# aiqm/torchani

Measured on AMD Instinct MI355X. Metric: atom*steps/sec (energy+forces) ANI-2x, higher is better.
Workload: dtype f32; 1 GPU; ANI-2x 8-member ensemble, 2336064-atom periodic water box (0.1 atoms/A^3), energy+forces, seeded random weights; n_atoms=2336064, shuffled_input=False, evaluated_on_cell_sorted_copy=False, two_product_backward=False

## Files before the change

torchani_amd/csrc/nbr.hip:

```cpp
#include "anihip_common.h"

namespace anihip {

struct GridDesc {
    double cell[9];
    double inv[9];
    double f0[3];
    double sc[3];
    float step[9];
    int nb[3];
    int range[3];
    int rep[3];
    int pbc[3];
    int ncell;
    unsigned lo_enc[3], hi_enc[3];
};

struct NbrWorkspace {
    GridDesc *desc;
    float4 *pos4;
    int *cellid;
    int *sorted_idx;
    float4 *pos4s;
    int *cell_start;
    int *cell_fill;
    int *scan_tmp;
};

static inline size_t align256(size_t x) { return (x + 255) & ~(size_t)255; }

static size_t carve(NbrWorkspace *w, char *base, int64_t n, int64_t max_cells)
{
    size_t off = 0;
    auto take = [&](size_t bytes) {
        char *p = base ? base + off : nullptr;
        off += align256(bytes);
        return p;
    };
    GridDesc *desc = (GridDesc *)take(sizeof(GridDesc));
    float4 *pos4 = (float4 *)take(sizeof(float4) * (size_t)n);
    int *cellid = (int *)take(sizeof(int) * (size_t)n);
    int *sorted_idx = (int *)take(sizeof(int) * (size_t)n);
    float4 *pos4s = (float4 *)take(sizeof(float4) * (size_t)n);
    int *cell_start = (int *)take(sizeof(int) * (size_t)(max_cells + 1));
    int *cell_fill = (int *)take(sizeof(int) * (size_t)(max_cells + 1));
    int *scan_tmp = (int *)take(sizeof(int) * (size_t)(max_cells / 1024 + 4));
    if (w) *w = NbrWorkspace{desc, pos4, cellid, sorted_idx, pos4s, cell_start, cell_fill, scan_tmp};
    return off;
}

__device__ __forceinline__ unsigned enc_f(float f)
{
    unsigned u = __float_as_uint(f);
    return (u & 0x80000000u) ? ~u : (u | 0x80000000u);
}
__device__ __forceinline__ float dec_f(unsigned e)
{
    unsigned u = (e & 0x80000000u) ? (e & 0x7FFFFFFFu) : ~e;
    return __uint_as_float(u);
}

__device__ void inv3(const double *m, double *o)
{
    double a = m[0], b = m[1], c = m[2], d = m[3], e = m[4], f = m[5], g = m[6], h = m[7], i = m[8];
    double det = a * (e * i - f * h) - b * (d * i - f * g) + c * (d * h - e * g);
    double id = 1.0 / det;
    o[0] = (e * i - f * h) * id; o[1] = (c * h - b * i) * id; o[2] = (b * f - c * e) * id;
    o[3] = (f * g - d * i) * id; o[4] = (a * i - c * g) * id; o[5] = (c * d - a * f) * id;
    o[6] = (d * h - e * g) * id; o[7] = (b * g - a * h) * id; o[8] = (a * e - b * d) * id;
}


__device__ void desc_fill(GridDesc *g, const float *cell, int pbc_mask, float cutoff)
{
    for (int q = 0; q < 9; ++q) g->cell[q] = cell ? (double)cell[q] : ((q % 4 == 0) ? 1.0 : 0.0);
    inv3(g->cell, g->inv);
    for (int k = 0; k < 3; ++k) {
        g->pbc[k] = (cell && ((pbc_mask >> k) & 1)) ? 1 : 0;
        double nrm = sqrt(g->inv[0 + k] * g->inv[0 + k] + g->inv[3 + k] * g->inv[3 + k] +
                          g->inv[6 + k] * g->inv[6 + k]);
        g->rep[k] = g->pbc[k] ? (int)ceil((double)cutoff * nrm) : 0;
        g->lo_enc[k] = 0xFFFFFFFFu;
        g->hi_enc[k] = 0u;
        g->f0[k] = 0.0;
        g->sc[k] = 1.0;
        g->nb[k] = 1;
        g->range[k] = 0;
    }
    g->ncell = 1;
}

__global__ void k_desc_init(GridDesc *g, const float *cell, int pbc_mask, float cutoff, uint32_t *status)
{
    if (blockIdx.x != 0) return;
    if (threadIdx.x < ANIHIP_STATUS_WORDS) status[threadIdx.x] = 0u;
    if (threadIdx.x == 0) desc_fill(g, cell, pbc_mask, cutoff);
}

__global__ void k_bbox(GridDesc *g, int64_t n, const int32_t *species, const float *coords)
{
    float lo[3] = {3.0e38f, 3.0e38f, 3.0e38f}, hi[3] = {-3.0e38f, -3.0e38f, -3.0e38f};
    for (int64_t i = blockIdx.x * (int64_t)blockDim.x + threadIdx.x; i < n;
         i += (int64_t)gridDim.x * blockDim.x) {
        if (species[i] < 0) continue;
        double x = coords[3 * i], y = coords[3 * i + 1], z = coords[3 * i + 2];
        for (int k = 0; k < 3; ++k) {
            float f = (float)(x * g->inv[0 + k] + y * g->inv[3 + k] + z * g->inv[6 + k]);
            lo[k] = fminf(lo[k], f);
            hi[k] = fmaxf(hi[k], f);
        }
    }
    for (int k = 0; k < 3; ++k) {
        for (int o = 32; o > 0; o >>= 1) {
            lo[k] = fminf(lo[k], __shfl_xor(lo[k], o));
            hi[k] = fmaxf(hi[k], __shfl_xor(hi[k], o));
        }
        if (lane_id() == 0) {
            atomicMin(&g->lo_enc[k], enc_f(lo[k]));
            atomicMax(&g->hi_enc[k], enc_f(hi[k]));
        }
    }
}

__global__ void k_grid_setup(GridDesc *g, float cutoff, int64_t max_cells, uint32_t *status)
{
    if (threadIdx.x != 0 || blockIdx.x != 0) return;
    double h[3], span[3];
    for (int k = 0; k < 3; ++k) {
        double nrm = sqrt(g->inv[0 + k] * g->inv[0 + k] + g->inv[3 + k] * g->inv[3 + k] +
                          g->inv[6 + k] * g->inv[6 + k]);
        h[k] = 1.0 / nrm;
        if (g->pbc[k]) {
            span[k] = 1.0;
            g->f0[k] = 0.0;
        } else {
            double lo = (double)dec_f(g->lo_enc[k]), hi = (double)dec_f(g->hi_enc[k]);
            if (!(hi >= lo)) { lo = 0.0; hi = 0.0; }
            double pad = 1e-4 * nrm + 1e-6 * (fabs(lo) + fabs(hi));
            lo -= pad; hi += pad;
            span[k] = hi - lo;
            g->f0[k] = lo;
        }
        int nb = (int)floor(span[k] * h[k] / (double)cutoff);
        g->nb[k] = nb < 1 ? 1 : nb;
    }
    bool coarsened = false;
    while ((int64_t)g->nb[0] * g->nb[1] * g->nb[2] > max_cells) {
        int k = 0;
        if (g->nb[1] > g->nb[k]) k = 1;
        if (g->nb[2] > g->nb[k]) k = 2;
        g->nb[k] = (g->nb[k] + 1) / 2;
        coarsened = true;
    }
    if (coarsened) atomicOr(&status[0], ANIHIP_ST_GRID_OVERFLOW);
    for (int k = 0; k < 3; ++k) {
        g->sc[k] = (double)g->nb[k] / span[k];
        double width = span[k] * h[k] / g->nb[k];
        g->range[k] = g->pbc[k] ? (int)ceil((double)cutoff / width) : 1;
        for (int q = 0; q < 3; ++q) g->step[3 * k + q] = (float)(g->cell[3 * k + q] / g->sc[k]);
    }
    g->ncell = g->nb[0] * g->nb[1] * g->nb[2];
    status[2] = (uint32_t)g->ncell;
}


__global__ void k_prep_batch(GridDesc *g, int64_t n, const int32_t *species, const float *coords, float4 *pos4,
                             const float *cell, int pbc_mask, float cutoff, uint32_t *status)
{
    if (blockIdx.x == 0) {
        if (threadIdx.x < ANIHIP_STATUS_WORDS) status[threadIdx.x] = 0u;
        if (threadIdx.x == 0) desc_fill(g, cell, pbc_mask, cutoff);
    }
    int64_t i = blockIdx.x * (int64_t)blockDim.x + threadIdx.x;
    if (i >= n) return;
    float x = coords[3 * i], y = coords[3 * i + 1], z = coords[3 * i + 2];
    if (cell && (pbc_mask & 7)) {
        double c[9], inv[9], f[3];
        for (int q = 0; q < 9; ++q) c[q] = (double)cell[q];
        inv3(c, inv);
        for (int k = 0; k < 3; ++k) {
            f[k] = (double)x * inv[0 + k] + (double)y * inv[3 + k] + (double)z * inv[6 + k];
            if ((pbc_mask >> k) & 1) f[k] -= floor(f[k]);
        }
        x = (float)(f[0] * c[0] + f[1] * c[3] + f[2] * c[6]);
        y = (float)(f[0] * c[1] + f[1] * c[4] + f[2] * c[7]);
        z = (float)(f[0] * c[2] + f[1] * c[5] + f[2] * c[8]);
    }
    int sp = species[i];
    uint32_t w = ((uint32_t)i & IDX_MASK) | ((sp < 0 ? SP_PAD : (uint32_t)sp) << 28);
    pos4[i] = make_float4(x, y, z, __uint_as_float(w));
}


__device__ __forceinline__ int wave_runs(int key, int &rank, int &head)
{
    const int lane = lane_id();
    const int k = key < 0 ? -1 - lane : key;
    const int prev = __shfl_up(k, 1);
    const bool is_head = lane == 0 || k != prev;
    const uint64_t heads = __ballot(is_head);
    const uint64_t below = heads & ((lane == 63) ? ~0ull : ((2ull << lane) - 1ull));
    head = 63 - (int)__builtin_clzll(below);
    rank = lane - head;
    const uint64_t above = lane == 63 ? 0ull : (heads >> (lane + 1));
    const int next = above ? lane + 1 + (int)__builtin_ctzll(above) : 64;
    return (is_head && key >= 0) ? next - lane : 0;
}

__global__ void k_bin_count(const GridDesc *g, int64_t n, const int32_t *species, const float *coords,
                            float4 *pos4, int *cellid, int *cell_cnt)
{
    int64_t i = blockIdx.x * (int64_t)blockDim.x + threadIdx.x;
    int c = -1;
    if (i < n) {
        int sp = species[i];
        if (sp >= 0) {
            double x = coords[3 * i], y = coords[3 * i + 1], z = coords[3 * i + 2];
            int b[3];
            double loc[3];
            for (int k = 0; k < 3; ++k) {
                double f = x * g->inv[0 + k] + y * g->inv[3 + k] + z * g->inv[6 + k];
                if (g->pbc[k]) f -= floor(f);
                double q = (f - g->f0[k]) * g->sc[k];
                int bk = (int)floor(q);
                bk = bk < 0 ? 0 : (bk >= g->nb[k] ? g->nb[k] - 1 : bk);
                b[k] = bk;
                loc[k] = (q - bk) / g->sc[k];
            }
            float ox = (float)(loc[0] * g->cell[0] + loc[1] * g->cell[3] + loc[2] * g->cell[6]);
            float oy = (float)(loc[0] * g->cell[1] + loc[1] * g->cell[4] + loc[2] * g->cell[7]);
            float oz = (float)(loc[0] * g->cell[2] + loc[1] * g->cell[5] + loc[2] * g->cell[8]);
            uint32_t w = ((uint32_t)i & IDX_MASK) | ((uint32_t)sp << 28);
            pos4[i] = make_float4(ox, oy, oz, __uint_as_float(w));
            c = (b[0] * g->nb[1] + b[1]) * g->nb[2] + b[2];
        }
        cellid[i] = c;
    }
    int rank, head;
    const int run = wave_runs(c, rank, head);
    if (run > 0) atomicAdd(&cell_cnt[c], run);
}

__global__ void k_scan_local(const GridDesc *g, const int *in, int *out, int *block_sums)
{
    __shared__ int s[1024];
    const int n = g->ncell;
    int i = blockIdx.x * 1024 + threadIdx.x;
    if (blockIdx.x * 1024 >= n + 1) return;
    int v = (i < n) ? in[i] : 0;
    s[threadIdx.x] = v;
    __syncthreads();
    for (int o = 1; o < 1024; o <<= 1) {
        int t = (threadIdx.x >= o) ? s[threadIdx.x - o] : 0;
        __syncthreads();
        s[threadIdx.x] += t;
        __syncthreads();
    }
    if (i <= n) out[i] = s[threadIdx.x] - v;
    if (threadIdx.x == 1023) block_sums[blockIdx.x] = s[1023];
}

__global__ __launch_bounds__(1024) void k_scan_top(const GridDesc *g, int *block_sums)
{
    __shared__ int s[1024];
    __shared__ int carry;
    if (blockIdx.x != 0) return;
    const int nblk = (g->ncell + 1 + 1023) / 1024;
    if (threadIdx.x == 0) carry = 0;
    __syncthreads();
    for (int base = 0; base < nblk; base += 1024) {
        const int i = base + (int)threadIdx.x;
        const int v = i < nblk ? block_sums[i] : 0;
        s[threadIdx.x] = v;
        __syncthreads();
        for (int o = 1; o < 1024; o <<= 1) {
            const int t = (threadIdx.x >= (unsigned)o) ? s[threadIdx.x - o] : 0;
            __syncthreads();
            s[threadIdx.x] += t;
            __syncthreads();
        }
        if (i < nblk) block_sums[i] = carry + s[threadIdx.x] - v;
        __syncthreads();
        if (threadIdx.x == 1023) carry += s[1023];
        __syncthreads();
    }
}

__global__ void k_scan_add(const GridDesc *g, int *out, const int *block_sums)
{
    int i = blockIdx.x * 1024 + threadIdx.x;
    if (i <= g->ncell) out[i] += block_sums[blockIdx.x];
}

__global__ void k_bin_fill(int64_t n, const int *cellid, const int *cell_start, int *cell_fill,
                           int *sorted_idx)
{
    int64_t i = blockIdx.x * (int64_t)blockDim.x + threadIdx.x;
    const int c = i < n ? cellid[i] : -1;
    int rank, head;
    const int run = wave_runs(c, rank, head);
    int base = 0;
    if (run > 0) base = atomicAdd(&cell_fill[c], run);
    base = __shfl(base, head);
    if (c >= 0) sorted_idx[cell_start[c] + base + rank] = (int)i;
}

__global__ void k_bin_rank_gather(int64_t n, const int *cellid, const int *cell_start, const int *sorted_idx,
                                  const float4 *pos4, float4 *pos4s)
{
    const int64_t i = blockIdx.x * (int64_t)blockDim.x + threadIdx.x;
    if (i >= n) return;
    const int c = cellid[i];
    if (c < 0) return;
    const int b = cell_start[c], e = cell_start[c + 1];
    int rank = 0;
    for (int p = b; p < e; ++p) rank += sorted_idx[p] < (int)i ? 1 : 0;
    pos4s[b + rank] = pos4[i];
}


constexpr int NBR_WPB = 4;

__device__ __forceinline__ int wrap_bin(int c, int nb)
{
    c = c < 0 ? c + nb : c;
    c = c >= nb ? c - nb : c;
    if (c < 0 || c >= nb) c = ((c % nb) + nb) % nb;
    return c;
}

struct HitList {
    float4 *buf;
    int n;
    bool overflow;
};

__device__ __forceinline__ void push_hits(HitList &h, bool hit, float dx, float dy, float dz, float w)
{
    uint64_t m = __ballot(hit);
    if (m == 0) return;
    int pos = h.n + mbcnt(m);
    if (hit && pos < MAXR) h.buf[pos] = make_float4(dx, dy, dz, w);
    h.n += __popcll(m);
    if (h.n > MAXR) {
        h.overflow = true;
        h.n = MAXR;
    }
}

__device__ void emit_row(HitList &h, int S, float rca2, int row_cap, uint32_t *meta_i, float4 *row,
                         uint32_t *status)
{
    wave_sync();
    const int lane = lane_id();
    int cnt[2][MAX_S];
#pragma unroll
    for (int g = 0; g < 2; ++g)
#pragma unroll
        for (int t = 0; t < MAX_S; ++t) cnt[g][t] = 0;
    const int n = h.n;
    for (int b0 = 0; b0 < n; b0 += WAVE) {
        int e = b0 + lane;
        bool v = e < n;
        float4 q = h.buf[v ? e : 0];
        int grp = (q.x * q.x + q.y * q.y + q.z * q.z <= rca2) ? 0 : 1;
        int sp = (int)(__float_as_uint(q.w) >> 28);
#pragma unroll
        for (int g = 0; g < 2; ++g)
#pragma unroll
            for (int t = 0; t < MAX_S; ++t)
                if (t < S) cnt[g][t] += __popcll(__ballot(v && grp == g && sp == t));
    }
    int nA = 0, nF = 0, mx = 0;
#pragma unroll
    for (int t = 0; t < MAX_S; ++t) {
        nA += cnt[0][t];
        nF += cnt[1][t];
        mx = max(mx, max(cnt[0][t], cnt[1][t]));
    }
    bool bad = h.overflow || (nA + nF > row_cap) || nA > MAXA || mx > 255;
    if (bad) {
// ... 56 lines not shown
        const size_t row0 = (size_t)(i - lo) * row_cap;
        if (lane == 0) meta_i[0] = (uint32_t)row0;
        const float4 pi = pos4[i];
        if ((__float_as_uint(pi.w) >> 28) == SP_PAD) {
            if (lane == 0) { meta_i[1] = 0; meta_i[2] = 0; meta_i[3] = 0; meta_i[4] = 0; meta_i[5] = 0; }
            continue;
        }
        HitList h{s_hits[wib], 0, false};
        const int64_t mol0 = (i / A) * A;
        for (int n0 = -r0; n0 <= r0; ++n0)
            for (int n1 = -r1; n1 <= r1; ++n1)
                for (int n2 = -r2; n2 <= r2; ++n2) {
                    const float sx = (float)(n0 * g->cell[0] + n1 * g->cell[3] + n2 * g->cell[6]);
                    const float sy = (float)(n0 * g->cell[1] + n1 * g->cell[4] + n2 * g->cell[7]);
                    const float sz = (float)(n0 * g->cell[2] + n1 * g->cell[5] + n2 * g->cell[8]);
                    const bool central_img = (n0 == 0 && n1 == 0 && n2 == 0);
                    for (int a0 = 0; a0 < A; a0 += WAVE) {
                        int a = a0 + lane;
                        bool v = a < A;
                        float4 c = pos4[mol0 + (v ? a : 0)];
                        float dx = (c.x + sx) - pi.x, dy = (c.y + sy) - pi.y, dz = (c.z + sz) - pi.z;
                        float d2 = dx * dx + dy * dy + dz * dz;
                        bool hit = v && ((__float_as_uint(c.w) >> 28) != SP_PAD) && d2 <= rcr2 &&
                                   !(central_img && (mol0 + a) == i);
                        push_hits(h, hit, dx, dy, dz, c.w);
                    }
                }
        emit_row(h, S, rca2, row_cap, meta_i, ent + row0, status);
        wave_sync();
    }
}

__global__ __launch_bounds__(NBR_WPB * WAVE) void k_nbr_cell(
    const GridDesc *g, int S, float rcr2, float rca2, int64_t lo, int64_t hi, const float4 *pos4,
    const int *cellid, const int *cell_start, const float4 *pos4s, int row_cap, uint32_t *meta,
    float4 *ent, uint32_t *status, const int *handled, const int *n_unhandled)
{
    if (n_unhandled && blockIdx.x == 0 && threadIdx.x == 0) status[3] = (uint32_t)*n_unhandled;
    if (n_unhandled && *n_unhandled == 0) return;
    __shared__ float4 s_hits[NBR_WPB][MAXR];
    __shared__ int s_pend[NBR_WPB][WAVE];
    __shared__ int s_k0[NBR_WPB][WAVE];
    __shared__ float4 s_shift[NBR_WPB][WAVE];
    const int wib = threadIdx.x >> 6, lane = lane_id();
    int *pend = s_pend[wib], *k0t = s_k0[wib];
    float4 *shift = s_shift[wib];
    const int64_t nw = (int64_t)gridDim.x * NBR_WPB;
    const int nb0 = g->nb[0], nb1 = g->nb[1], nb2 = g->nb[2];
    const int R0 = g->range[0], R1 = g->range[1], R2 = g->range[2];
    const int p0 = g->pbc[0], p1 = g->pbc[1], p2 = g->pbc[2];
    float st[9];
#pragma unroll
    for (int q = 0; q < 9; ++q) st[q] = g->step[q];
    const int n1 = 2 * R1 + 1, n2 = 2 * R2 + 1, ncells = (2 * R0 + 1) * n1 * n2;
    const float inv_n2 = 1.0f / (float)n2, inv_n1 = 1.0f / (float)n1;
    for (int64_t i = lo + blockIdx.x * (int64_t)NBR_WPB + wib; i < hi; i += nw) {
        uint32_t *meta_i = meta + (size_t)i * META_W;
        const size_t row0 = (size_t)(i - lo) * row_cap;
        if (lane == 0) meta_i[0] = (uint32_t)row0;
        const int c = cellid[i];
        if (c < 0) {
            if (lane == 0) { meta_i[1] = 0; meta_i[2] = 0; meta_i[3] = 0; meta_i[4] = 0; meta_i[5] = 0; }
            continue;
        }
        if (handled && handled[c]) continue;
        const float4 pi = pos4[i];
        const int cu = uniform(c);
        const int b2 = cu % nb2, b1 = (cu / nb2) % nb1, b0 = cu / (nb2 * nb1);
        HitList h{s_hits[wib], 0, false};
        for (int cb = 0; cb < ncells; cb += WAVE) {
            const int ci = cb + lane;
            const int q2 = (int)(((float)ci + 0.5f) * inv_n2);
            const int q1 = (int)(((float)q2 + 0.5f) * inv_n1);
            const int o2 = ci - q2 * n2 - R2, o1 = q2 - q1 * n1 - R1, o0 = q1 - R0;
            int c0 = b0 + o0, c1 = b1 + o1, c2 = b2 + o2;
            bool ok = ci < ncells;
            if (p0) c0 = wrap_bin(c0, nb0); else ok = ok && c0 >= 0 && c0 < nb0;
            if (p1) c1 = wrap_bin(c1, nb1); else ok = ok && c1 >= 0 && c1 < nb1;
            if (p2) c2 = wrap_bin(c2, nb2); else ok = ok && c2 >= 0 && c2 < nb2;
            const int cw = ok ? (c0 * nb1 + c1) * nb2 + c2 : 0;
            const int kbeg = cell_start[cw], kend = cell_start[cw + 1];
            const int cnt = ok ? kend - kbeg : 0;
            int incl = cnt;
#pragma unroll
            for (int d = 1; d < WAVE; d <<= 1) {
                const int up = __shfl_up(incl, d);
                incl += lane >= d ? up : 0;
            }
            const int total = __builtin_amdgcn_readlane(incl, WAVE - 1);
            pend[lane] = incl;
            k0t[lane] = kbeg - (incl - cnt);
            shift[lane] = make_float4(o0 * st[0] + o1 * st[3], o0 * st[1] + o1 * st[4], o0 * st[2] + o1 * st[5],
                                      __int_as_float((o2 + 512) | ((o0 == 0 && o1 == 0 && o2 == 0) ? 1024 : 0)));
            wave_sync();
            for (int x0 = 0; x0 < total; x0 += WAVE) {
                const int x = x0 + lane;
                const bool v = x < total;
                int seg = 0;
#pragma unroll
                for (int stp = WAVE / 2; stp > 0; stp >>= 1) seg += pend[seg + stp - 1] <= x ? stp : 0;
                seg = seg < WAVE ? seg : WAVE - 1;
                const int k = v ? x + k0t[seg] : 0;
                const float4 cnd = pos4s[k];
                const float4 sh = shift[seg];
                const int code = __float_as_int(sh.w);
                const int o2s = (code & 1023) - 512;
                const float dx = cnd.x + (sh.x - pi.x) + o2s * st[6];
                const float dy = cnd.y + (sh.y - pi.y) + o2s * st[7];
                const float dz = cnd.z + (sh.z - pi.z) + o2s * st[8];
                const float d2 = dx * dx + dy * dy + dz * dz;
                const bool self = (code & 1024) && ((__float_as_uint(cnd.w) & IDX_MASK) == ((uint32_t)i & IDX_MASK));
                const bool hit = v && d2 <= rcr2 && !self;
                push_hits(h, hit, dx, dy, dz, cnd.w);
            }
            wave_sync();
        }
        emit_row(h, S, rca2, row_cap, meta_i, ent + row0, status);
        wave_sync();
    }
}

template <bool WIDE>
__device__ __forceinline__ int byte_sum(uint64_t p)
{
    if constexpr (WIDE) {
        const uint64_t h = (p & 0x00FF00FF00FF00FFull) + ((p >> 8) & 0x00FF00FF00FF00FFull);
        return (int)((h * 0x0001000100010001ull) >> 48);
    } else {
        return (int)((p * 0x0101010101010101ull) >> 56);
    }
}

template <int NAT, int NCH>
__device__ __forceinline__ void emit_from_stage(const float4 *cand, const uint16_t *hidx, const int (&nh_)[NAT],
// ... 71 lines not shown
            uint2 *m2 = reinterpret_cast<uint2 *>(meta_i);
            m2[0] = make_uint2((uint32_t)row0, bad ? 0u : ((uint32_t)nA | ((uint32_t)nF << 16)));
            m2[1] = bad ? make_uint2(0u, 0u) : make_uint2((uint32_t)pk[t][0], (uint32_t)(pk[t][0] >> 32));
            m2[2] = bad ? make_uint2(0u, 0u) : make_uint2((uint32_t)pk[t][1], (uint32_t)(pk[t][1] >> 32));
        }
    }
}

constexpr int NBR2_WPB = 16;
constexpr int CAND_CAP = 448;
#ifdef ANIHIP_TRACE
__device__ unsigned long long g_nbr_trace[1024][10];
#define NTR_STAMP(k_)                                                      \
    {                                                                      \
        const unsigned long long now_ = __builtin_amdgcn_s_memtime();      \
        if (wib == 0) tr_sum[k_] += now_ - tr_last;                        \
        tr_last = now_;                                                    \
    }
#else
#define NTR_STAMP(k_)
#endif

__device__ __forceinline__ uint32_t wave_or(uint32_t v)
{
#pragma unroll
    for (int o = 32; o > 0; o >>= 1) v |= (uint32_t)__shfl_xor((int)v, o);
    return v;
}

__global__ __launch_bounds__(NBR2_WPB * WAVE, 4) void k_nbr_cell2(
    const GridDesc *g, int S, float rcr2, float rca2, int64_t lo, int64_t hi, const int *cellid,
    const int *cell_start, const float4 *pos4s, int row_cap, uint32_t *meta, float4 *ent, uint32_t *status,
    int *handled, int *n_unhandled)
{
    __shared__ float4 s_cand[NBR2_WPB][CAND_CAP];
    __shared__ uint16_t s_hidx[NBR2_WPB][2 * MAXR];
    static_assert(2 * MAXR * sizeof(uint16_t) >= 2 * WAVE * sizeof(int), "staging tables share the hit list's LDS");
    const int wib = threadIdx.x >> 6, lane = lane_id();
    float4 *cand = s_cand[wib];
    uint16_t *hidx = s_hidx[wib];
    int *pend = reinterpret_cast<int *>(s_hidx[wib]), *k0t = pend + WAVE;
    for (int64_t i = lo + blockIdx.x * (int64_t)blockDim.x + threadIdx.x; i < hi; i += (int64_t)gridDim.x * blockDim.x)
        if (cellid[i] < 0) {
            uint32_t *m = meta + (size_t)i * META_W;
            m[0] = (uint32_t)((size_t)(i - lo) * row_cap);
            m[1] = 0; m[2] = 0; m[3] = 0; m[4] = 0; m[5] = 0;
        }
    const int nb0 = g->nb[0], nb1 = g->nb[1], nb2 = g->nb[2];
    const int R0 = g->range[0], R1 = g->range[1], R2 = g->range[2];
    const int p0 = g->pbc[0], p1 = g->pbc[1], p2 = g->pbc[2];
    float st[9];
#pragma unroll
    for (int q = 0; q < 9; ++q) st[q] = g->step[q];
    const int n1 = 2 * R1 + 1, n2 = 2 * R2 + 1, ncells = (2 * R0 + 1) * n1 * n2;
    const float inv_n2 = 1.0f / (float)n2, inv_n1 = 1.0f / (float)n1;
    const int nbins = nb0 * nb1 * nb2;
    const int nw = gridDim.x * NBR2_WPB;
    __shared__ uint32_t s_queue;
    if (threadIdx.x == 0) s_queue = NBR2_WPB;
    __syncthreads();
    auto bin_at = [&](uint32_t p) { return (int)(p / NBR2_WPB) * nw + (int)blockIdx.x * NBR2_WPB + (int)(p % NBR2_WPB); };
    uint32_t qv = 0u;
#ifdef ANIHIP_TRACE
    unsigned long long tr_sum[10] = {0, 0, 0, 0, 0, 0, 0, 0, 0, 0}, tr_last = __builtin_amdgcn_s_memtime();
#endif
    for (int c = bin_at(wib); c < nbins; c = bin_at((uint32_t)__builtin_amdgcn_readfirstlane((int)qv))) {
        if (lane == 0) qv = atomicAdd(&s_queue, 1u);
        NTR_STAMP(0)
        const int ab = cell_start[c], ae = cell_start[c + 1];
        if (ae == ab) continue;
#ifdef ANIHIP_TRACE
        if (wib == 0) tr_sum[8] += 1;
#endif
        bool mine = false;
        for (int a0 = ab; a0 < ae; a0 += WAVE) {
            const int a = a0 + lane;
            const int64_t ia = a < ae ? (int64_t)(__float_as_uint(pos4s[a].w) & IDX_MASK) : -1;
            mine = mine || __ballot(ia >= lo && ia < hi) != 0ull;
        }
        if (!mine) continue;
        const int b2 = c % nb2, b1 = (c / nb2) % nb1, b0 = c / (nb2 * nb1);
        int total = 0, self_base = 0;
        if (ncells <= WAVE) {
            const int ci = lane;
            const int q2 = (int)(((float)ci + 0.5f) * inv_n2);
            const int q1 = (int)(((float)q2 + 0.5f) * inv_n1);
            const int o2 = ci - q2 * n2 - R2, o1 = q2 - q1 * n1 - R1, o0 = q1 - R0;
            int c0 = b0 + o0, c1 = b1 + o1, c2 = b2 + o2;
            bool ok = ci < ncells;
            if (p0) c0 = wrap_bin(c0, nb0); else ok = ok && c0 >= 0 && c0 < nb0;
            if (p1) c1 = wrap_bin(c1, nb1); else ok = ok && c1 >= 0 && c1 < nb1;
            if (p2) c2 = wrap_bin(c2, nb2); else ok = ok && c2 >= 0 && c2 < nb2;
            const int cw = ok ? (c0 * nb1 + c1) * nb2 + c2 : 0;
            const int kbeg = cell_start[cw], kend = cell_start[cw + 1];
            const int cnt = ok ? kend - kbeg : 0;
            int incl = cnt;
#pragma unroll
            for (int d = 1; d < WAVE; d <<= 1) {
                const int up = __shfl_up(incl, d);
                incl += lane >= d ? up : 0;
            }
            total = __builtin_amdgcn_readlane(incl, WAVE - 1);
            pend[lane] = incl;
            k0t[lane] = kbeg - (incl - cnt);
            const bool central = ok && o0 == 0 && o1 == 0 && o2 == 0;
            const uint64_t cm = __ballot(central);
            self_base = __builtin_amdgcn_readlane(incl - cnt, (int)__builtin_ctzll(cm | (1ull << 63)));
        }
        const bool fits = ncells <= WAVE && total <= CAND_CAP;
        if (lane == 0) {
            handled[c] = fits ? 1 : 0;
            if (!fits) atomicAdd(n_unhandled, 1);
        }
        if (!fits) continue;
        wave_sync();
        NTR_STAMP(1)
        {
            constexpr int NST = CAND_CAP / WAVE;
            float4 qs[NST];
#pragma unroll
            for (int it = 0; it < NST; ++it) {
                const int x = it * WAVE + lane;
                qs[it] = make_float4(0.f, 0.f, 0.f, 0.f);
                if (it * WAVE < total) {
                    const int xc = x < total ? x : total - 1;
                    int seg = 0;
#pragma unroll
                    for (int stp = WAVE / 2; stp > 0; stp >>= 1) seg += pend[seg + stp - 1] <= xc ? stp : 0;
                    seg = seg < WAVE ? seg : WAVE - 1;
                    const float4 q = pos4s[xc + k0t[seg]];
                    const int q2 = (int)(((float)seg + 0.5f) * inv_n2);
                    const int q1 = (int)(((float)q2 + 0.5f) * inv_n1);
                    const int o2 = seg - q2 * n2 - R2, o1 = q2 - q1 * n1 - R1, o0 = q1 - R0;
                    qs[it] = make_float4(q.x + (o0 * st[0] + o1 * st[3] + o2 * st[6]), q.y + (o0 * st[1] + o1 * st[4] + o2 * st[7]),
                                         q.z + (o0 * st[2] + o1 * st[5] + o2 * st[8]), q.w);
                }
            }
#pragma unroll
            for (int it = 0; it < NST; ++it)
                if (it * WAVE + lane < total) cand[it * WAVE + lane] = qs[it];
        }
        uint32_t cls_mask = 0u;
        wave_sync();
        for (int x0 = 0; x0 < total; x0 += WAVE)
            cls_mask |= (x0 + lane < total) ? 1u << (__float_as_uint(cand[x0 + lane].w) >> 28) : 0u;
        cls_mask = wave_or(cls_mask);
        cls_mask = __builtin_amdgcn_readfirstlane(cls_mask | (cls_mask << 8));
        NTR_STAMP(2)
        for (int a = ab; a < ae; a += 2) {
            const int xa = self_base + (a - ab), xb = xa + 1;
            const float4 pa = cand[xa];
            const float4 pb = cand[a + 1 < ae ? xb : xa];
            const int64_t ia = (int64_t)((uint32_t)uniform((int)__float_as_uint(pa.w)) & IDX_MASK);
            const int64_t ib = (int64_t)((uint32_t)uniform((int)__float_as_uint(pb.w)) & IDX_MASK);
            const bool da = ia >= lo && ia < hi, db = a + 1 < ae && ib >= lo && ib < hi;
            if (!da && !db) continue;
            int nha = 0, nhb = 0;
            float4 q = cand[lane < total ? lane : 0];
            for (int x0 = 0; x0 < total; x0 += WAVE) {
                const int x = x0 + lane, xn = x + WAVE;
                const float4 qn = cand[xn < total ? xn : 0];
                const float ax = q.x - pa.x, ay = q.y - pa.y, az = q.z - pa.z;
                const float bx = q.x - pb.x, by = q.y - pb.y, bz = q.z - pb.z;
                const float d2a = ax * ax + ay * ay + az * az, d2b = bx * bx + by * by + bz * bz;
                const bool inr = x < total;
                const bool hita = (int)da & (int)inr & (int)(d2a <= rcr2) & (int)(x != xa);
                const bool hitb = (int)db & (int)inr & (int)(d2b <= rcr2) & (int)(x != xb);
                const uint64_t ma = __ballot(hita), mb = __ballot(hitb);
                const int posa = nha + mbcnt(ma), posb = nhb + mbcnt(mb);
                if ((int)hita & (int)(posa < MAXR)) hidx[posa] = (uint16_t)x;
                if ((int)hitb & (int)(posb < MAXR)) hidx[MAXR + posb] = (uint16_t)x;
                nha += __popcll(ma);
                nhb += __popcll(mb);
                q = qn;
            }
            wave_sync();
            NTR_STAMP(3)
            {
                const int nh2[2] = {nha, nhb};
                const bool act2[2] = {da, db};
                const float4 p2[2] = {pa, pb};
                const int64_t i2[2] = {ia, ib};
                if (max(nha, nhb) <= 2 * WAVE) {
                    emit_from_stage<2, 2>(cand, hidx, nh2, act2, p2, i2, lo, row_cap, rca2, cls_mask, meta, ent, status);
                } else {
                    {
                        const int nh1[1] = {nha};
                        const bool act1[1] = {da};
                        const float4 p1[1] = {pa};
                        const int64_t i1[1] = {ia};
                        emit_from_stage<1, MAXR / WAVE>(cand, hidx, nh1, act1, p1, i1, lo, row_cap, rca2, cls_mask, meta, ent,
                                                        status);
                    }
                    {
                        const int nh1[1] = {nhb};
                        const bool act1[1] = {db};
                        const float4 p1[1] = {pb};
                        const int64_t i1[1] = {ib};
                        emit_from_stage<1, MAXR / WAVE>(cand, hidx + MAXR, nh1, act1, p1, i1, lo, row_cap, rca2, cls_mask, meta,
                                                        ent, status);
                    }
                }
            }
            wave_sync();
            NTR_STAMP(4)
        }
        wave_sync();
    }
#ifdef ANIHIP_TRACE
    if (wib == 0 && lane == 0 && blockIdx.x < 1024)
        for (int q_ = 0; q_ < 10; ++q_) g_nbr_trace[blockIdx.x][q_] = tr_sum[q_];
#endif
}

__global__ __launch_bounds__(NBR_WPB * WAVE) void k_nbr_full(int S, float rcr2, float rca2, int64_t n_atoms,
                                                            const int32_t *species, const float *coords,
                                                            int64_t n_i, const int32_t *ilist,
                                                            const int32_t *numneigh, const int64_t *start,
// ... 158 lines not shown
    int64_t b = (n_central + NBR_WPB - 1) / NBR_WPB;
    if (b < 1) b = 1;
    if (b > 256 * 16) b = 256 * 16;
    return (int)b;
}

extern "C" int anihip_nbr_build_batch(void *stream_, const anihip_aev_params *p, int32_t n_mol,
                                      int32_t A, const int32_t *species, const float *coords,
                                      const float *cell, int32_t pbc_mask, int64_t lo, int64_t hi,
                                      void *workspace, size_t workspace_bytes, uint32_t *meta, float *ent,
                                      int64_t ent_capacity, uint32_t *status)
{
    hipStream_t stream = (hipStream_t)stream_;
    const int64_t n = (int64_t)n_mol * A;
    ANIHIP_REQUIRE(p && species && coords && workspace && meta && ent && status, "null pointer argument");
    ANIHIP_REQUIRE(p->num_species >= 1 && p->num_species <= MAX_S - 1, "num_species must be 1..7");
    ANIHIP_REQUIRE(0 <= lo && lo <= hi && hi <= n, "central range [%lld,%lld) outside 0..%lld",
                   (long long)lo, (long long)hi, (long long)n);
    ANIHIP_REQUIRE(n < (int64_t)IDX_MASK, "too many atoms for 28-bit neighbor indices");
    ANIHIP_REQUIRE(workspace_bytes >= anihip_nbr_workspace_bytes(n, 1), "workspace too small");
    if (hi == lo) return 0;
    const int64_t row_cap = ent_capacity / (hi - lo);
    ANIHIP_REQUIRE(row_cap >= 1 && (hi - lo) * row_cap < ((int64_t)1 << 32), "bad ent_capacity");
    NbrWorkspace w;
    carve(&w, (char *)workspace, n, 1);
    hipLaunchKernelGGL(k_prep_batch, dim3((unsigned)((n + 255) / 256)), dim3(256), 0, stream, w.desc, n,
                       species, coords, w.pos4, cell, pbc_mask, p->Rcr, status);
    hipLaunchKernelGGL(k_nbr_batch, dim3(nbr_grid_blocks(hi - lo)), dim3(NBR_WPB * WAVE), 0, stream,
                       w.desc, p->num_species, p->Rcr * p->Rcr, p->Rca * p->Rca, (int)A, lo, hi, w.pos4,
                       (int)(row_cap > MAXR ? MAXR : row_cap), meta, (float4 *)ent, status);
    ANIHIP_CHECK_HIP(hipGetLastError());
    return 0;
}

extern "C" int anihip_nbr_build_cell(void *stream_, const anihip_aev_params *p, int64_t n,
                                     const int32_t *species, const float *coords, const float *cell,
                                     int32_t pbc_mask, int64_t lo, int64_t hi, int64_t max_cells,
                                     void *workspace, size_t workspace_bytes, uint32_t *meta, float *ent,
                                     int64_t ent_capacity, uint32_t *status)
{
    hipStream_t stream = (hipStream_t)stream_;
    ANIHIP_REQUIRE(p && species && coords && workspace && meta && ent && status, "null pointer argument");
    ANIHIP_REQUIRE(p->num_species >= 1 && p->num_species <= MAX_S - 1, "num_species must be 1..7");
    ANIHIP_REQUIRE(0 <= lo && lo <= hi && hi <= n, "central range outside 0..n");
    ANIHIP_REQUIRE(n < (int64_t)IDX_MASK, "too many atoms for 28-bit neighbor indices");
    ANIHIP_REQUIRE(max_cells >= 1 && max_cells < ((int64_t)1 << 30), "bad max_cells");
    ANIHIP_REQUIRE(workspace_bytes >= anihip_nbr_workspace_bytes(n, max_cells), "workspace too small");
    if (hi == lo) return 0;
    const int64_t row_cap = ent_capacity / (hi - lo);
    ANIHIP_REQUIRE(row_cap >= 1 && (hi - lo) * row_cap < ((int64_t)1 << 32), "bad ent_capacity");
    NbrWorkspace w;
    carve(&w, (char *)workspace, n, max_cells);
    const unsigned nblk = (unsigned)((n + 255) / 256);
    const unsigned cblk = (unsigned)((max_cells + 1 + 1023) / 1024);
    hipLaunchKernelGGL(k_desc_init, dim3(1), dim3(64), 0, stream, w.desc, cell, pbc_mask, p->Rcr, status);
    const bool all_pbc = cell && ((pbc_mask & 7) == 7);
    if (!all_pbc)
        hipLaunchKernelGGL(k_bbox, dim3(nblk > 1024 ? 1024 : nblk), dim3(256), 0, stream, w.desc, n,
                           species, coords);
    hipLaunchKernelGGL(k_grid_setup, dim3(1), dim3(64), 0, stream, w.desc, p->Rcr, max_cells, status);
    zero_words_async(stream, w.cell_fill, sizeof(int) * (size_t)(max_cells + 1));
    hipLaunchKernelGGL(k_bin_count, dim3(nblk), dim3(256), 0, stream, w.desc, n, species, coords, w.pos4,
                       w.cellid, w.cell_fill);
    hipLaunchKernelGGL(k_scan_local, dim3(cblk), dim3(1024), 0, stream, w.desc, w.cell_fill, w.cell_start,
                       w.scan_tmp);
    hipLaunchKernelGGL(k_scan_top, dim3(1), dim3(1024), 0, stream, w.desc, w.scan_tmp);
    hipLaunchKernelGGL(k_scan_add, dim3(cblk), dim3(1024), 0, stream, w.desc, w.cell_start, w.scan_tmp);
    zero_words_async(stream, w.cell_fill, sizeof(int) * (size_t)(max_cells + 1));
    hipLaunchKernelGGL(k_bin_fill, dim3(nblk), dim3(256), 0, stream, n, w.cellid, w.cell_start, w.cell_fill,
                       w.sorted_idx);
    hipLaunchKernelGGL(k_bin_rank_gather, dim3(nblk), dim3(256), 0, stream, n, w.cellid, w.cell_start, w.sorted_idx,
                       w.pos4, w.pos4s);
    int *handled = w.cell_fill, *n_unhandled = w.scan_tmp;
    zero_words_async(stream, n_unhandled, sizeof(int));
    const int rc = (int)(row_cap > MAXR ? MAXR : row_cap);
    int64_t bins_blocks = (max_cells + NBR2_WPB - 1) / NBR2_WPB;
    if (bins_blocks > 256) bins_blocks = 256;
    hipLaunchKernelGGL(k_nbr_cell2, dim3((unsigned)bins_blocks), dim3(NBR2_WPB * WAVE), 0, stream, w.desc,
                       p->num_species, p->Rcr * p->Rcr, p->Rca * p->Rca, lo, hi, w.cellid, w.cell_start, w.pos4s, rc,
                       meta, (float4 *)ent, status, handled, n_unhandled);
    hipLaunchKernelGGL(k_nbr_cell, dim3(nbr_grid_blocks(hi - lo)), dim3(NBR_WPB * WAVE), 0, stream, w.desc,
                       p->num_species, p->Rcr * p->Rcr, p->Rca * p->Rca, lo, hi, w.pos4, w.cellid,
                       w.cell_start, w.pos4s, rc, meta, (float4 *)ent, status, handled, n_unhandled);
    ANIHIP_CHECK_HIP(hipGetLastError());
    return 0;
}

extern "C" size_t anihip_nbr_half_workspace_bytes(int64_t n_central)
{
    return align256(sizeof(int) * (size_t)(n_central > 0 ? n_central : 1));
}

extern "C" int anihip_nbr_from_half(void *stream_, const anihip_aev_params *p, int64_t n, const int32_t *species,
                                    int64_t n_pairs, const int64_t *idx, const float *diff, int64_t lo,
                                    int64_t hi, void *workspace, size_t workspace_bytes, uint32_t *meta,
                                    float *ent, int64_t ent_capacity, uint32_t *status)
{
    hipStream_t stream = (hipStream_t)stream_;
    ANIHIP_REQUIRE(p && species && workspace && meta && ent && status, "null pointer argument");
    ANIHIP_REQUIRE(n_pairs == 0 || (idx && diff), "null neighbor list");
    ANIHIP_REQUIRE(p->num_species >= 1 && p->num_species <= MAX_S - 1, "num_species must be 1..7");
    ANIHIP_REQUIRE(0 <= lo && lo <= hi && hi <= n, "central range outside 0..n");
    ANIHIP_REQUIRE(n < (int64_t)IDX_MASK, "too many atoms for 28-bit neighbor indices");
    ANIHIP_REQUIRE(n_pairs >= 0, "negative pair count");
    ANIHIP_REQUIRE(workspace_bytes >= anihip_nbr_half_workspace_bytes(hi - lo), "workspace too small");
    if (hi == lo) return 0;
    const int64_t row_cap = ent_capacity / (hi - lo);
    ANIHIP_REQUIRE(row_cap >= 1 && (hi - lo) * row_cap < ((int64_t)1 << 32), "bad ent_capacity");
    const int cap = (int)(row_cap > MAXR ? MAXR : row_cap);
    int *count = (int *)workspace;
    zero_words_async(stream, count, sizeof(int) * (size_t)(hi - lo));
    if (n_pairs > 0) {
        int64_t blocks = (n_pairs + 255) / 256;
        if (blocks > 256 * 32) blocks = 256 * 32;
        hipLaunchKernelGGL(k_half_scatter, dim3((unsigned)blocks), dim3(256), 0, stream, n_pairs, idx, diff, species,
                           n, p->Rcr * p->Rcr, lo, hi, cap, count, (float4 *)ent, status);
    }
    hipLaunchKernelGGL(k_half_finish, dim3(nbr_grid_blocks(hi - lo)), dim3(NBR_WPB * WAVE), 0, stream,
                       p->num_species, p->Rca * p->Rca, lo, hi, species, cap, count, meta, (float4 *)ent, status);
    ANIHIP_CHECK_HIP(hipGetLastError());
    return 0;
}

__device__ __forceinline__ bool half_keep(int64_t i, const float4 e)
{
    const int64_t j = (int64_t)(__float_as_uint(e.w) & IDX_MASK);
    if (j != i) return j > i;
    return e.x > 0.f || (e.x == 0.f && (e.y > 0.f || (e.y == 0.f && e.z > 0.f)));
}

__global__ __launch_bounds__(256) void k_half_count(int64_t lo, int64_t hi, const uint32_t *meta, const float4 *ent,
                                                   int64_t *counts)
{
// ... 168 lines not shown
```

Measured before the change: 75.56 million atom*steps/s.

## Split cells into x half-cells to narrow candidate scan in cell-pair neighbor search

```diff
diff --git a/torchani_amd/csrc/nbr.hip b/torchani_amd/csrc/nbr.hip
--- a/torchani_amd/csrc/nbr.hip
+++ b/torchani_amd/csrc/nbr.hip
@@ -14,6 +14,7 @@
     int pbc[3];
     int ncell;
     unsigned lo_enc[3], hi_enc[3];
+    int limit0;
 };
 
 struct NbrWorkspace {
@@ -42,9 +43,9 @@
     int *cellid = (int *)take(sizeof(int) * (size_t)n);
     int *sorted_idx = (int *)take(sizeof(int) * (size_t)n);
     float4 *pos4s = (float4 *)take(sizeof(float4) * (size_t)n);
-    int *cell_start = (int *)take(sizeof(int) * (size_t)(max_cells + 1));
-    int *cell_fill = (int *)take(sizeof(int) * (size_t)(max_cells + 1));
-    int *scan_tmp = (int *)take(sizeof(int) * (size_t)(max_cells / 1024 + 4));
+    int *cell_start = (int *)take(sizeof(int) * (size_t)(2 * max_cells + 2));
+    int *cell_fill = (int *)take(sizeof(int) * (size_t)(2 * max_cells + 2));
+    int *scan_tmp = (int *)take(sizeof(int) * (size_t)(2 * max_cells / 1024 + 4));
     if (w) *w = NbrWorkspace{desc, pos4, cellid, sorted_idx, pos4s, cell_start, cell_fill, scan_tmp};
     return off;
 }
@@ -88,13 +89,7 @@
         g->range[k] = 0;
     }
     g->ncell = 1;
-}
-
-__global__ void k_desc_init(GridDesc *g, const float *cell, int pbc_mask, float cutoff, uint32_t *status)
-{
-    if (blockIdx.x != 0) return;
-    if (threadIdx.x < ANIHIP_STATUS_WORDS) status[threadIdx.x] = 0u;
-    if (threadIdx.x == 0) desc_fill(g, cell, pbc_mask, cutoff);
+    g->limit0 = 0;
 }
 
 __global__ void k_bbox(GridDesc *g, int64_t n, const int32_t *species, const float *coords)
@@ -122,9 +117,8 @@
     }
 }
 
-__global__ void k_grid_setup(GridDesc *g, float cutoff, int64_t max_cells, uint32_t *status)
-{
-    if (threadIdx.x != 0 || blockIdx.x != 0) return;
+__device__ void grid_setup(GridDesc *g, float cutoff, int64_t max_cells, uint32_t *status)
+{
     double h[3], span[3];
     for (int k = 0; k < 3; ++k) {
         double nrm = sqrt(g->inv[0 + k] * g->inv[0 + k] + g->inv[3 + k] * g->inv[3 + k] +
@@ -157,10 +151,25 @@
         g->sc[k] = (double)g->nb[k] / span[k];
         double width = span[k] * h[k] / g->nb[k];
         g->range[k] = g->pbc[k] ? (int)ceil((double)cutoff / width) : 1;
+        if (k == 0) g->limit0 = (g->range[0] == 1 && width >= (double)cutoff * (1.0 + 1e-4)) ? 1 : 0;
         for (int q = 0; q < 3; ++q) g->step[3 * k + q] = (float)(g->cell[3 * k + q] / g->sc[k]);
     }
     g->ncell = g->nb[0] * g->nb[1] * g->nb[2];
     status[2] = (uint32_t)g->ncell;
+}
+
+__global__ void k_grid_setup(GridDesc *g, float cutoff, int64_t max_cells, uint32_t *status)
+{
+    if (threadIdx.x != 0 || blockIdx.x != 0) return;
+    grid_setup(g, cutoff, max_cells, status);
+}
+
+__global__ void k_desc_init(GridDesc *g, const float *cell, int pbc_mask, float cutoff, int64_t max_cells, uint32_t *status)
+{
+    if (blockIdx.x != 0 || threadIdx.x != 0) return;
+    for (int q = 0; q < ANIHIP_STATUS_WORDS; ++q) status[q] = 0u;
+    desc_fill(g, cell, pbc_mask, cutoff);
+    if (max_cells > 0) grid_setup(g, cutoff, max_cells, status);
 }
 
 
@@ -216,7 +225,7 @@
         int sp = species[i];
         if (sp >= 0) {
             double x = coords[3 * i], y = coords[3 * i + 1], z = coords[3 * i + 2];
-            int b[3];
+            int b[3], upper = 0;
             double loc[3];
             for (int k = 0; k < 3; ++k) {
                 double f = x * g->inv[0 + k] + y * g->inv[3 + k] + z * g->inv[6 + k];
@@ -225,6 +234,7 @@
                 int bk = (int)floor(q);
                 bk = bk < 0 ? 0 : (bk >= g->nb[k] ? g->nb[k] - 1 : bk);
                 b[k] = bk;
+                if (k == 0) upper = (q - bk) * 2.0 >= 1.0 ? 1 : 0;
                 loc[k] = (q - bk) / g->sc[k];
             }
             float ox = (float)(loc[0] * g->cell[0] + loc[1] * g->cell[3] + loc[2] * g->cell[6]);
@@ -232,7 +242,7 @@
             float oz = (float)(loc[0] * g->cell[2] + loc[1] * g->cell[5] + loc[2] * g->cell[8]);
             uint32_t w = ((uint32_t)i & IDX_MASK) | ((uint32_t)sp << 28);
             pos4[i] = make_float4(ox, oy, oz, __uint_as_float(w));
-            c = (b[0] * g->nb[1] + b[1]) * g->nb[2] + b[2];
+            c = 2 * ((b[0] * g->nb[1] + b[1]) * g->nb[2] + b[2]) + upper;
         }
         cellid[i] = c;
     }
@@ -244,7 +254,7 @@
 __global__ void k_scan_local(const GridDesc *g, const int *in, int *out, int *block_sums)
 {
     __shared__ int s[1024];
-    const int n = g->ncell;
+    const int n = 2 * g->ncell;
     int i = blockIdx.x * 1024 + threadIdx.x;
     if (blockIdx.x * 1024 >= n + 1) return;
     int v = (i < n) ? in[i] : 0;
@@ -265,7 +275,7 @@
     __shared__ int s[1024];
     __shared__ int carry;
     if (blockIdx.x != 0) return;
-    const int nblk = (g->ncell + 1 + 1023) / 1024;
+    const int nblk = (2 * g->ncell + 1 + 1023) / 1024;
     if (threadIdx.x == 0) carry = 0;
     __syncthreads();
     for (int base = 0; base < nblk; base += 1024) {
@@ -286,10 +296,13 @@
     }
 }
 
-__global__ void k_scan_add(const GridDesc *g, int *out, const int *block_sums)
+__global__ void k_scan_add(const GridDesc *g, int *out, const int *block_sums, int *counters)
 {
     int i = blockIdx.x * 1024 + threadIdx.x;
-    if (i <= g->ncell) out[i] += block_sums[blockIdx.x];
+    if (i <= 2 * g->ncell) {
+        out[i] += block_sums[blockIdx.x];
+        counters[i] = 0;
+    }
 }
 
 __global__ void k_bin_fill(int64_t n, const int *cellid, const int *cell_start, int *cell_fill,
@@ -327,6 +340,17 @@
     c = c >= nb ? c - nb : c;
     if (c < 0 || c >= nb) c = ((c % nb) + nb) % nb;
     return c;
+}
+
+__device__ __forceinline__ void stencil_lane(int ci, bool split, int n1, int n2, float inv_n1, float inv_n2, int R0, int R1,
+                                             int R2, int &o0, int &o1, int &o2, int &upper)
+{
+    const int q2 = (int)(((float)ci + 0.5f) * inv_n2);
+    const int q1 = (int)(((float)q2 + 0.5f) * inv_n1);
+    o2 = ci - q2 * n2 - R2;
+    o1 = q2 - q1 * n1 - R1;
+    upper = split ? (q1 & 1) : 0;
+    o0 = (split ? (q1 >> 1) : q1) - R0;
 }
 
 struct HitList {
@@ -489,13 +513,15 @@
     float st[9];
 #pragma unroll
     for (int q = 0; q < 9; ++q) st[q] = g->step[q];
-    const int n1 = 2 * R1 + 1, n2 = 2 * R2 + 1, ncells = (2 * R0 + 1) * n1 * n2;
+    const int n1 = 2 * R1 + 1, n2 = 2 * R2 + 1;
+    const bool split = 2 * (2 * R0 + 1) * n1 * n2 <= WAVE;
+    const int ncells = (split ? 2 : 1) * (2 * R0 + 1) * n1 * n2;
     const float inv_n2 = 1.0f / (float)n2, inv_n1 = 1.0f / (float)n1;
     for (int64_t i = lo + blockIdx.x * (int64_t)NBR_WPB + wib; i < hi; i += nw) {
         uint32_t *meta_i = meta + (size_t)i * META_W;
         const size_t row0 = (size_t)(i - lo) * row_cap;
         if (lane == 0) meta_i[0] = (uint32_t)row0;
-        const int c = cellid[i];
+        const int c = cellid[i] >> 1;
         if (c < 0) {
             if (lane == 0) { meta_i[1] = 0; meta_i[2] = 0; meta_i[3] = 0; meta_i[4] = 0; meta_i[5] = 0; }
             continue;
@@ -507,16 +533,15 @@
         HitList h{s_hits[wib], 0, false};
         for (int cb = 0; cb < ncells; cb += WAVE) {
             const int ci = cb + lane;
-            const int q2 = (int)(((float)ci + 0.5f) * inv_n2);
-            const int q1 = (int)(((float)q2 + 0.5f) * inv_n1);
-            const int o2 = ci - q2 * n2 - R2, o1 = q2 - q1 * n1 - R1, o0 = q1 - R0;
+            int o0, o1, o2, upper;
+            stencil_lane(ci, split, n1, n2, inv_n1, inv_n2, R0, R1, R2, o0, o1, o2, upper);
             int c0 = b0 + o0, c1 = b1 + o1, c2 = b2 + o2;
             bool ok = ci < ncells;
             if (p0) c0 = wrap_bin(c0, nb0); else ok = ok && c0 >= 0 && c0 < nb0;
             if (p1) c1 = wrap_bin(c1, nb1); else ok = ok && c1 >= 0 && c1 < nb1;
             if (p2) c2 = wrap_bin(c2, nb2); else ok = ok && c2 >= 0 && c2 < nb2;
             const int cw = ok ? (c0 * nb1 + c1) * nb2 + c2 : 0;
-            const int kbeg = cell_start[cw], kend = cell_start[cw + 1];
+            const int kbeg = cell_start[2 * cw + upper], kend = cell_start[2 * cw + (split ? upper + 1 : 2)];
             const int cnt = ok ? kend - kbeg : 0;
             int incl = cnt;
 #pragma unroll
@@ -694,7 +719,10 @@
     float st[9];
 #pragma unroll
     for (int q = 0; q < 9; ++q) st[q] = g->step[q];
-    const int n1 = 2 * R1 + 1, n2 = 2 * R2 + 1, ncells = (2 * R0 + 1) * n1 * n2;
+    const int n1 = 2 * R1 + 1, n2 = 2 * R2 + 1;
+    const bool split = 2 * (2 * R0 + 1) * n1 * n2 <= WAVE;
+    const int ncells = (split ? 2 : 1) * (2 * R0 + 1) * n1 * n2;
+    const bool limit = split && g->limit0 != 0;
     const float inv_n2 = 1.0f / (float)n2, inv_n1 = 1.0f / (float)n1;
     const int nbins = nb0 * nb1 * nb2;
     const int nw = gridDim.x * NBR2_WPB;
@@ -709,7 +737,7 @@
     for (int c = bin_at(wib); c < nbins; c = bin_at((uint32_t)__builtin_amdgcn_readfirstlane((int)qv))) {
         if (lane == 0) qv = atomicAdd(&s_queue, 1u);
         NTR_STAMP(0)
-        const int ab = cell_start[c], ae = cell_start[c + 1];
+        const int ab = cell_start[2 * c], am = cell_start[2 * c + 1], ae = cell_start[2 * c + 2];
         if (ae == ab) continue;
 #ifdef ANIHIP_TRACE
         if (wib == 0) tr_sum[8] += 1;
@@ -722,19 +750,18 @@
         }
         if (!mine) continue;
         const int b2 = c % nb2, b1 = (c / nb2) % nb1, b0 = c / (nb2 * nb1);
-        int total = 0, self_base = 0;
+        int total = 0, self_base = 0, self_upper = 0, x_lo = 0, x_hi = 0;
         if (ncells <= WAVE) {
             const int ci = lane;
-            const int q2 = (int)(((float)ci + 0.5f) * inv_n2);
-            const int q1 = (int)(((float)q2 + 0.5f) * inv_n1);
-            const int o2 = ci - q2 * n2 - R2, o1 = q2 - q1 * n1 - R1, o0 = q1 - R0;
+            int o0, o1, o2, upper;
+            stencil_lane(ci, split, n1, n2, inv_n1, inv_n2, R0, R1, R2, o0, o1, o2, upper);
             int c0 = b0 + o0, c1 = b1 + o1, c2 = b2 + o2;
             bool ok = ci < ncells;
             if (p0) c0 = wrap_bin(c0, nb0); else ok = ok && c0 >= 0 && c0 < nb0;
             if (p1) c1 = wrap_bin(c1, nb1); else ok = ok && c1 >= 0 && c1 < nb1;
             if (p2) c2 = wrap_bin(c2, nb2); else ok = ok && c2 >= 0 && c2 < nb2;
             const int cw = ok ? (c0 * nb1 + c1) * nb2 + c2 : 0;
-            const int kbeg = cell_start[cw], kend = cell_start[cw + 1];
+            const int kbeg = cell_start[2 * cw + upper], kend = cell_start[2 * cw + (split ? upper + 1 : 2)];
             const int cnt = ok ? kend - kbeg : 0;
             int incl = cnt;
 #pragma unroll
@@ -746,8 +773,11 @@
             pend[lane] = incl;
             k0t[lane] = kbeg - (incl - cnt);
             const bool central = ok && o0 == 0 && o1 == 0 && o2 == 0;
-            const uint64_t cm = __ballot(central);
+            const uint64_t cm = __ballot(central && upper == 0), cu = __ballot(central && upper == 1);
             self_base = __builtin_amdgcn_readlane(incl - cnt, (int)__builtin_ctzll(cm | (1ull << 63)));
+            self_upper = __builtin_amdgcn_readlane(incl - cnt, (int)__builtin_ctzll(cu | (1ull << 63)));
+            x_lo = limit ? __builtin_amdgcn_readlane(incl - cnt, limit ? n1 * n2 : 0) : 0;
+            x_hi = limit ? __builtin_amdgcn_readlane(incl - cnt, limit ? 5 * n1 * n2 : 0) : total;
         }
         const bool fits = ncells <= WAVE && total <= CAND_CAP;
         if (lane == 0) {
@@ -771,9 +801,8 @@
                     for (int stp = WAVE / 2; stp > 0; stp >>= 1) seg += pend[seg + stp - 1] <= xc ? stp : 0;
                     seg = seg < WAVE ? seg : WAVE - 1;
                     const float4 q = pos4s[xc + k0t[seg]];
-                    const int q2 = (int)(((float)seg + 0.5f) * inv_n2);
-                    const int q1 = (int)(((float)q2 + 0.5f) * inv_n1);
-                    const int o2 = seg - q2 * n2 - R2, o1 = q2 - q1 * n1 - R1, o0 = q1 - R0;
+                    int o0, o1, o2, upper;
+                    stencil_lane(seg, split, n1, n2, inv_n1, inv_n2, R0, R1, R2, o0, o1, o2, upper);
                     qs[it] = make_float4(q.x + (o0 * st[0] + o1 * st[3] + o2 * st[6]), q.y + (o0 * st[1] + o1 * st[4] + o2 * st[7]),
                                          q.z + (o0 * st[2] + o1 * st[5] + o2 * st[8]), q.w);
                 }
@@ -790,7 +819,10 @@
         cls_mask = __builtin_amdgcn_readfirstlane(cls_mask | (cls_mask << 8));
         NTR_STAMP(2)
         for (int a = ab; a < ae; a += 2) {
-            const int xa = self_base + (a - ab), xb = xa + 1;
+            const bool ua = split && a >= am, ub = a + 1 < ae ? split && a + 1 >= am : ua;
+            const int xa = ua ? self_upper + (a - am) : self_base + (a - ab);
+            const int xb = a + 1 < ae ? (ub ? self_upper + (a + 1 - am) : self_base + (a + 1 - ab)) : xa + 1;
+            const int xs = ua ? x_lo : 0, xe = ub ? total : x_hi;
             const float4 pa = cand[xa];
             const float4 pb = cand[a + 1 < ae ? xb : xa];
             const int64_t ia = (int64_t)((uint32_t)uniform((int)__float_as_uint(pa.w)) & IDX_MASK);
@@ -798,14 +830,14 @@
             const bool da = ia >= lo && ia < hi, db = a + 1 < ae && ib >= lo && ib < hi;
             if (!da && !db) continue;
             int nha = 0, nhb = 0;
-            float4 q = cand[lane < total ? lane : 0];
-            for (int x0 = 0; x0 < total; x0 += WAVE) {
+            float4 q = cand[xs + lane < xe ? xs + lane : 0];
+            for (int x0 = xs; x0 < xe; x0 += WAVE) {
                 const int x = x0 + lane, xn = x + WAVE;
-                const float4 qn = cand[xn < total ? xn : 0];
+                const float4 qn = cand[xn < xe ? xn : 0];
                 const float ax = q.x - pa.x, ay = q.y - pa.y, az = q.z - pa.z;
                 const float bx = q.x - pb.x, by = q.y - pb.y, bz = q.z - pb.z;
                 const float d2a = ax * ax + ay * ay + az * az, d2b = bx * bx + by * by + bz * bz;
-                const bool inr = x < total;
+                const bool inr = x < xe;
                 const bool hita = (int)da & (int)inr & (int)(d2a <= rcr2) & (int)(x != xa);
                 const bool hitb = (int)db & (int)inr & (int)(d2b <= rcr2) & (int)(x != xb);
                 const uint64_t ma = __ballot(hita), mb = __ballot(hitb);
@@ -1070,33 +1102,40 @@
     NbrWorkspace w;
     carve(&w, (char *)workspace, n, max_cells);
     const unsigned nblk = (unsigned)((n + 255) / 256);
-    const unsigned cblk = (unsigned)((max_cells + 1 + 1023) / 1024);
-    hipLaunchKernelGGL(k_desc_init, dim3(1), dim3(64), 0, stream, w.desc, cell, pbc_mask, p->Rcr, status);
+    const unsigned cblk = (unsigned)((2 * max_cells + 1 + 1023) / 1024);
     const bool all_pbc = cell && ((pbc_mask & 7) == 7);
-    if (!all_pbc)
+    hipLaunchKernelGGL(k_desc_init, dim3(1), dim3(64), 0, stream, w.desc, cell, pbc_mask, p->Rcr,
+                       all_pbc ? max_cells : (int64_t)0, status);
+    if (!all_pbc) {
         hipLaunchKernelGGL(k_bbox, dim3(nblk > 1024 ? 1024 : nblk), dim3(256), 0, stream, w.desc, n,
                            species, coords);
-    hipLaunchKernelGGL(k_grid_setup, dim3(1), dim3(64), 0, stream, w.desc, p->Rcr, max_cells, status);
-    zero_words_async(stream, w.cell_fill, sizeof(int) * (size_t)(max_cells + 1));
+        hipLaunchKernelGGL(k_grid_setup, dim3(1), dim3(64), 0, stream, w.desc, p->Rcr, max_cells, status);
+    }
+    zero_words_async(stream, w.cell_fill, sizeof(int) * (size_t)(2 * max_cells + 1));
     hipLaunchKernelGGL(k_bin_count, dim3(nblk), dim3(256), 0, stream, w.desc, n, species, coords, w.pos4,
                        w.cellid, w.cell_fill);
     hipLaunchKernelGGL(k_scan_local, dim3(cblk), dim3(1024), 0, stream, w.desc, w.cell_fill, w.cell_start,
                        w.scan_tmp);
     hipLaunchKernelGGL(k_scan_top, dim3(1), dim3(1024), 0, stream, w.desc, w.scan_tmp);
-    hipLaunchKernelGGL(k_scan_add, dim3(cblk), dim3(1024), 0, stream, w.desc, w.cell_start, w.scan_tmp);
-    zero_words_async(stream, w.cell_fill, sizeof(int) * (size_t)(max_cells + 1));
+    hipLaunchKernelGGL(k_scan_add, dim3(cblk), dim3(1024), 0, stream, w.desc, w.cell_start, w.scan_tmp, w.cell_fill);
     hipLaunchKernelGGL(k_bin_fill, dim3(nblk), dim3(256), 0, stream, n, w.cellid, w.cell_start, w.cell_fill,
                        w.sorted_idx);
     hipLaunchKernelGGL(k_bin_rank_gather, dim3(nblk), dim3(256), 0, stream, n, w.cellid, w.cell_start, w.sorted_idx,
                        w.pos4, w.pos4s);
     int *handled = w.cell_fill, *n_unhandled = w.scan_tmp;
-    zero_words_async(stream, n_unhandled, sizeof(int));
     const int rc = (int)(row_cap > MAXR ? MAXR : row_cap);
-    int64_t bins_blocks = (max_cells + NBR2_WPB - 1) / NBR2_WPB;
-    if (bins_blocks > 256) bins_blocks = 256;
-    hipLaunchKernelGGL(k_nbr_cell2, dim3((unsigned)bins_blocks), dim3(NBR2_WPB * WAVE), 0, stream, w.desc,
-                       p->num_species, p->Rcr * p->Rcr, p->Rca * p->Rca, lo, hi, w.cellid, w.cell_start, w.pos4s, rc,
-                       meta, (float4 *)ent, status, handled, n_unhandled);
+    const char *per_atom = getenv("ANIHIP_NBR_PER_ATOM");
+    if (per_atom && per_atom[0] == '1') {
+        handled = nullptr;
+        n_unhandled = nullptr;
+    } else {
+        zero_words_async(stream, n_unhandled, sizeof(int));
+        int64_t bins_blocks = (max_cells + NBR2_WPB - 1) / NBR2_WPB;
+        if (bins_blocks > 256) bins_blocks = 256;
+        hipLaunchKernelGGL(k_nbr_cell2, dim3((unsigned)bins_blocks), dim3(NBR2_WPB * WAVE), 0, stream, w.desc,
+                           p->num_species, p->Rcr * p->Rcr, p->Rca * p->Rca, lo, hi, w.cellid, w.cell_start, w.pos4s, rc,
+                           meta, (float4 *)ent, status, handled, n_unhandled);
+    }
     hipLaunchKernelGGL(k_nbr_cell, dim3(nbr_grid_blocks(hi - lo)), dim3(NBR_WPB * WAVE), 0, stream, w.desc,
                        p->num_species, p->Rcr * p->Rcr, p->Rca * p->Rca, lo, hi, w.pos4, w.cellid,
                        w.cell_start, w.pos4s, rc, meta, (float4 *)ent, status, handled, n_unhandled);
```

Result: no change. 75.65 million atom*steps/s, median of 5 (+0.1%).
